# gebegebegebe/onnx-transformer

Measured on AMD Instinct MI355X. Metric: decoded tokens/sec IWSLT14 de-en int8 greedy (batch 32 over 1 GPU, 71 steps), higher is better.
Workload: dtype int8; 1 GPU; cfg2: greedy decode, src<=64 padded to 72, max_len=72, 32 sentences length-sorted over 1 rank(s); global_batch=32, per_gpu_batch=32, seq_len=72, parallelism=sentence-shard x1

## Files before the change

onnx-transformer_amd/csrc/qtx_decode.hip:

```cpp
#include <cstdlib>

#include "qtx_common.h"
#include "qtx_kernels.h"
#include "qtx_knobs.h"

QTX_STAMP_SETTER(decode)

namespace qtx {

__device__ __forceinline__ uint4 unpack_i4(uint2 h) {
  auto sext = [](uint32_t v) { return v | ((v & 0x08080808u) * 0x1Eu); };
  const uint32_t lo0 = sext(h.x & 0x0F0F0F0Fu), hi0 = sext((h.x >> 4) & 0x0F0F0F0Fu);
  const uint32_t lo1 = sext(h.y & 0x0F0F0F0Fu), hi1 = sext((h.y >> 4) & 0x0F0F0F0Fu);
  uint4 o;
  o.x = __builtin_amdgcn_perm(hi0, lo0, 0x05010400u);
  o.y = __builtin_amdgcn_perm(hi0, lo0, 0x07030602u);
  o.z = __builtin_amdgcn_perm(hi1, lo1, 0x05010400u);
  o.w = __builtin_amdgcn_perm(hi1, lo1, 0x07030602u);
  return o;
}

template <int RB, int K, int AMODE, class F>
__device__ __forceinline__ void skinny_prologue(const SkinnyArgs& g, uint8_t* As, float* sas,
                                                int m0, int tid, int wave, int lane,
                                                F&& issue_rest) {
  constexpr int LDA = K + 16;
  constexpr int BM = RB <= 16 ? 16 : 32;
  constexpr int RPW = RB / 4;
  if constexpr (AMODE == A_I8) {
    constexpr int CPR = K / 16, TOT = RB * CPR, NLD = (TOT + 255) / 256;
    uint4 v[NLD];
#pragma unroll
    for (int j = 0; j < NLD; ++j) {
      const int idx = min(tid + 256 * j, TOT - 1), m = min(m0 + idx / CPR, g.M - 1);
      v[j] = ld_at(reinterpret_cast<const uint4*>(g.A), (unsigned)(m * K + 16 * (idx % CPR)));
    }
    issue_rest();
    if (tid < BM) sas[tid] = (tid < RB && m0 + tid < g.M) ? g.sa[m0 + tid] : 0.0f;
#pragma unroll
    for (int j = 0; j < NLD; ++j) {
      const int idx = tid + 256 * j, r = idx / CPR;
      if (TOT % 256 == 0 || idx < TOT)
        *reinterpret_cast<uint4*>(As + r * LDA + 16 * (idx % CPR)) =
            (m0 + r < g.M) ? v[j] : make_uint4(0, 0, 0, 0);
// ... 69 lines not shown
        uint32_t* dst = reinterpret_cast<uint32_t*>(As + r * LDA);
        float tf[4 * NC];
#pragma unroll
        for (int c = 0; c < NC; ++c) {
          tf[4 * c] = t[jb][c].x; tf[4 * c + 1] = t[jb][c].y;
          tf[4 * c + 2] = t[jb][c].z; tf[4 * c + 3] = t[jb][c].w;
        }
        uint32_t qd[NC];
#if defined(QTX_ABL) && (QTX_ABL & 8)
#pragma unroll
        for (int c = 0; c < NC; ++c) qd[c] = __float_as_uint(tf[4 * c] * sc);
#else
        quant_pack<4 * NC>(tf, sc, qd);
#endif
#pragma unroll
        for (int c = 0; c < NC; ++c) dst[lane + 64 * c] = ok ? qd[c] : 0u;
        if (lane == 0) sas[r] = ok ? sc : 0.0f;
      }
    }
  }
}

template <int MF, int RB, int K, int WBITS, int AMODE, int FLAGS>
__global__ __launch_bounds__(256) void k_skinny(SkinnyArgs g) {
  constexpr int BM = 16 * MF;
  static_assert(RB % 4 == 0 && RB <= BM, "rows per block");
  constexpr int KW = K / 4;
  constexpr int NS = KW / 64;
  constexpr int LDA = K + 16;
  __shared__ __attribute__((aligned(16))) uint8_t As[BM * LDA];
  __shared__ float sas[BM];
  __shared__ v4i red[4][MF][64];

  const int tid = threadIdx.x, wave = tid >> 6, lane = tid & 63;
  const int fr = lane & 15, fg = lane >> 4;
  const int n0 = blockIdx.x * 16, m0 = blockIdx.y * RB;

  QTX_STAMP(0);

  const int n = min(n0 + fr, g.N - 1);
  uint4 wf[NS];
  uint2 wp[NS];
  const int col = n0 + fr;
  const bool cok = col < g.N;
  float swc = 0.0f, bc = 0.0f, rv[MF];
  constexpr bool resid = FLAGS & EPI_RESIDUAL;
  auto issue_rest = [&]() {
#pragma unroll
    for (int s = 0; s < NS; ++s) {
      const int k = wave * KW + 64 * s + 16 * fg;
#if defined(QTX_ABL) && (QTX_ABL & 1)
      wf[s] = make_uint4(n + k, k, n, 1); wp[s] = make_uint2(n, k);
#else
      if constexpr (WBITS == 8)
        wf[s] = ld_at(reinterpret_cast<const uint4*>(g.W), (unsigned)(n * (int)g.ldw + k));
      else
        wp[s] = ld_at(reinterpret_cast<const uint2*>(g.W), (unsigned)(n * (int)g.ldw + (k >> 1)));
#endif
    }
    const int cc = min(col, g.N - 1);
    swc = ld_at(g.sw, 4u * cc);
    bc = ld_at(g.bias, 4u * cc);
    if constexpr (resid) {
#pragma unroll
      for (int i = 0; i < MF; ++i) {
        const int row = min(m0 + 16 * i + 4 * fg + wave, g.M - 1);
        rv[i] = ld_at(g.res, 4u * (unsigned)(row * (int)g.ldr + cc));
      }
    }
  };

  skinny_prologue<RB, K, AMODE>(g, As, sas, m0, tid, wave, lane, issue_rest);
  __syncthreads();

  QTX_STAMP(1);
  v4i acc[MF];
#pragma unroll
  for (int i = 0; i < MF; ++i) acc[i] = v4i{0, 0, 0, 0};
#pragma unroll
  for (int s = 0; s < NS; ++s) {
    v4i bfr;
    if constexpr (WBITS == 8) {
      bfr = __builtin_bit_cast(v4i, wf[s]);
    } else {
      bfr = __builtin_bit_cast(v4i, unpack_i4(wp[s]));
    }
    const int k = wave * KW + 64 * s + 16 * fg;
#pragma unroll
    for (int i = 0; i < MF; ++i) {
      const v4i afr = *reinterpret_cast<const v4i*>(As + (16 * i + fr) * LDA + k);
#if defined(QTX_ABL) && (QTX_ABL & 4)
      acc[i] += afr ^ bfr;
// ... 15 lines not shown
      int sum = 0;
#pragma unroll
      for (int w = 0; w < 4; ++w) sum += reinterpret_cast<const int*>(&red[w][i][lane])[e];
      const int r = 16 * i + 4 * fg + e, row = m0 + r;
      const bool ok = cok && r < RB && row < g.M;
      float y = ((float)sum * sas[r]) * swc + bc;
      if constexpr (relu) y = y > 0.0f ? y : 0.0f;
      if constexpr (resid) y = rv[i] + y;
      if (ok) st_at(g.out, 4u * (unsigned)(row * (int)g.ldo + col), y);
      if constexpr (rmax) {
        float am = ok ? fabsf(y) : 0.0f;
        am = fmaxf(am, dpp<0xB1>(am));
        am = fmaxf(am, dpp<0x4E>(am));
        am = fmaxf(am, dpp<0x141>(am));
        am = fmaxf(am, dpp<0x140>(am));
        if (fr == 0 && r < RB && row < g.M) g.pmax_out[(long)blockIdx.x * g.M + row] = am;
      }
    }
  }
  QTX_STAMP(3);
}

template <bool OWN>
__global__ __launch_bounds__(512) void k_skinny8_ffn2(SkinnyArgs g) {
  constexpr int K = 2048, RB = 4, KW = K / 8, NS = KW / 64, LDA = K + 16;
  __shared__ __attribute__((aligned(16))) uint8_t As[16 * LDA];
  __shared__ float sas[16];
  __shared__ v4i red[8][64];
  __shared__ float hmax[8];
  const int tid = threadIdx.x, wave = tid >> 6, lane = tid & 63;
  const int fr = lane & 15, fg = lane >> 4;
  const int n0 = blockIdx.x * 16, m0 = blockIdx.y * RB;
  const int r = wave >> 1, half = wave & 1;
  const int m = min(m0 + r, g.M - 1);
  float4 t[4];
#pragma unroll
  for (int c = 0; c < 4; ++c)
    t[c] = ld_at(reinterpret_cast<const float4*>(g.X), 4u * (unsigned)(m * (int)g.ldx + 4 * (lane + 64 * (4 * half + c))));
  float pm[2] = {0.0f, 0.0f};
  if constexpr (!OWN)
#pragma unroll
    for (int u = 0; u < 2; ++u) pm[u] = ld_at(g.pmax_in, 4u * (unsigned)(min(lane + 64 * u, g.pmax_n - 1) * g.M + m));
  const int n = min(n0 + fr, g.N - 1);
  uint4 wf[NS];
#pragma unroll
  for (int s = 0; s < NS; ++s)
    wf[s] = ld_at(reinterpret_cast<const uint4*>(g.W), (unsigned)(n * (int)g.ldw + wave * KW + 64 * s + 16 * fg));
  const int col = n0 + fr, cc = min(col, g.N - 1);
  const bool cok = col < g.N;
  const float swc = ld_at(g.sw, 4u * cc), bc = ld_at(g.bias, 4u * cc);
  const float rv = ld_at(g.res, 4u * (unsigned)(min(m0 + fg, g.M - 1) * (int)g.ldr + cc));
  {
    const bool ok = m0 + r < g.M;
    float rmax;
    if constexpr (OWN) {
      float lm = 0.0f;
#pragma unroll
      for (int c = 0; c < 4; ++c)
        lm = fmaxf(lm, fmaxf(fmaxf(fabsf(t[c].x), fabsf(t[c].y)), fmaxf(fabsf(t[c].z), fabsf(t[c].w))));
      lm = wave_max(lm);
      if (lane == 0) hmax[wave] = lm;
      __syncthreads();
      rmax = fmaxf(hmax[2 * r], hmax[2 * r + 1]);
    } else {
      rmax = wave_max(fmaxf(pm[0], pm[1]));
    }
    const float sc = quant_scale(rmax, 127.0f);
    float tf[16];
#pragma unroll
    for (int c = 0; c < 4; ++c) {
      tf[4 * c] = t[c].x; tf[4 * c + 1] = t[c].y; tf[4 * c + 2] = t[c].z; tf[4 * c + 3] = t[c].w;
    }
    uint32_t qd[4];
    quant_pack<16>(tf, sc, qd);
// ... 4 lines not shown
  }
  __syncthreads();
  v4i acc = v4i{0, 0, 0, 0};
#pragma unroll
  for (int s = 0; s < NS; ++s) {
    const v4i afr = *reinterpret_cast<const v4i*>(As + fr * LDA + wave * KW + 64 * s + 16 * fg);
    acc = __builtin_amdgcn_mfma_i32_16x16x64_i8(afr, __builtin_bit_cast(v4i, wf[s]), acc, 0, 0, 0);
  }
  red[wave][lane] = acc;
  __syncthreads();
  if (wave != 0) return;
  {
    const int e = fg, src = fr;
    int sum = 0;
#pragma unroll
    for (int w = 0; w < 8; ++w) sum += reinterpret_cast<const int*>(&red[w][src])[e];
    const int row = m0 + e;
    const float y = ((float)sum * sas[e]) * swc + bc;
    if (cok && row < g.M) st_at(g.out, 4u * (unsigned)(row * (int)g.ldo + col), rv + y);
  }
}

template <int RB, int WBITS, int AMODE, int FLAGS>
__global__ __launch_bounds__(256) void k_skinny_wide(SkinnyArgs g) {
  constexpr int K = 512, NS = K / 64, LDA = K + 16;
  static_assert(RB % 4 == 0 && RB <= 16, "rows per block");
  __shared__ __attribute__((aligned(16))) uint8_t As[16 * LDA];
  __shared__ float sas[16];
  constexpr int RPL = RB / 4;
  constexpr bool REMAP = RB == 4 || RB == 8;
  __shared__ v4i tail[REMAP ? 4 : 1][REMAP ? 4 * RB : 1];
  const int tid = threadIdx.x, wave = tid >> 6, lane = tid & 63;
  const int fr = lane & 15, fg = lane >> 4;
  const int n0 = blockIdx.x * 64 + 16 * wave, m0 = blockIdx.y * RB;
  QTX_STAMP(0);
  const int n = min(n0 + fr, g.N - 1);
  uint4 wf[NS];
  uint2 wp[NS];
  const int col = n0 + fr;
  const bool cok = col < g.N;
  constexpr bool resid = FLAGS & EPI_RESIDUAL;
  float swc, bc, rv[4];
  auto issue_rest = [&]() {
#pragma unroll
    for (int s = 0; s < NS; ++s) {
      const int k = 64 * s + 16 * fg;
#if defined(QTX_ABL) && (QTX_ABL & 1)
      wf[s] = make_uint4(n + k, k, n, 1); wp[s] = make_uint2(n, k);
#else
      if constexpr (WBITS == 8)
        wf[s] = ld_at(reinterpret_cast<const uint4*>(g.W), (unsigned)(n * (int)g.ldw + k));
      else
        wp[s] = ld_at(reinterpret_cast<const uint2*>(g.W), (unsigned)(n * (int)g.ldw + (k >> 1)));
#endif
    }
    swc = cok ? ld_at(g.sw, 4u * col) : 0.0f;
    bc = cok ? ld_at(g.bias, 4u * col) : 0.0f;
    if constexpr (RB == 4) {
      rv[0] = (resid && cok && m0 + fg < g.M) ? ld_at(g.res, 4u * (unsigned)((m0 + fg) * (int)g.ldr + col)) : 0.0f;
    } else if constexpr (RB == 8) {
#pragma unroll
      for (int j = 0; j < 2; ++j) {
        const int row = m0 + fg + 4 * j;
        rv[j] = (resid && cok && row < g.M) ? ld_at(g.res, 4u * (unsigned)(row * (int)g.ldr + col)) : 0.0f;
      }
    } else {
#pragma unroll
      for (int e = 0; e < 4; ++e) {
        const int r = 4 * fg + e, row = m0 + r;
        rv[e] = (resid && cok && r < RB && row < g.M) ? ld_at(g.res, 4u * (unsigned)(row * (int)g.ldr + col)) : 0.0f;
      }
    }
  };
  skinny_prologue<RB, K, AMODE>(g, As, sas, m0, tid, wave, lane, issue_rest);
  __syncthreads();
  QTX_STAMP(1);
  v4i acc = v4i{0, 0, 0, 0};
#pragma unroll
  for (int s = 0; s < NS; ++s) {
// ... 58 lines not shown
  for (int e = 0; e < 4; ++e) {
    const int r = 4 * fg + e, row = m0 + r;
    const bool ok = cok && r < RB && row < g.M;
    float y = ((float)acc[e] * sas[r]) * swc + bc;
    if constexpr (relu) y = y > 0.0f ? y : 0.0f;
    if constexpr (resid) y = rv[e] + y;
    if (ok) st_at(g.out, 4u * (unsigned)(row * (int)g.ldo + col), y);
    if constexpr (rmax) {
      float am = ok ? fabsf(y) : 0.0f;
      am = fmaxf(am, dpp<0xB1>(am));
      am = fmaxf(am, dpp<0x4E>(am));
      am = fmaxf(am, dpp<0x141>(am));
      am = fmaxf(am, dpp<0x140>(am));
      if (fr == 0 && r < RB && row < g.M) g.pmax_out[(long)(n0 >> 4) * g.M + row] = am;
    }
  }
  QTX_STAMP(3);
}

template <int RB, int WB, int AM>
hipError_t skinny_wide_flags(const SkinnyArgs& g, hipStream_t st) {
  const dim3 grid(g.N / 64, (g.M + RB - 1) / RB);
  switch (g.flags) {
    case 0: k_skinny_wide<RB, WB, AM, 0><<<grid, 256, 0, st>>>(g); break;
    case EPI_RELU: k_skinny_wide<RB, WB, AM, EPI_RELU><<<grid, 256, 0, st>>>(g); break;
    case EPI_RESIDUAL: k_skinny_wide<RB, WB, AM, EPI_RESIDUAL><<<grid, 256, 0, st>>>(g); break;
    case EPI_RELU | EPI_ROWMAX:
      k_skinny_wide<RB, WB, AM, EPI_RELU | EPI_ROWMAX><<<grid, 256, 0, st>>>(g);
      break;
    default: return hipErrorInvalidValue;
  }
  return hipGetLastError();
}
template <int WB, int AM>
hipError_t skinny_wide_rb(const SkinnyArgs& g, int rb, hipStream_t st) {
  switch (rb) {
    case 4: return skinny_wide_flags<4, WB, AM>(g, st);
    case 8: return skinny_wide_flags<8, WB, AM>(g, st);
    case 16: return skinny_wide_flags<16, WB, AM>(g, st);
    default: return hipErrorInvalidValue;
  }
}

template <int MF, int RB, int K, int WB, int AM>
hipError_t skinny_flags(const SkinnyArgs& g, hipStream_t st) {
  const dim3 grid(g.N / 16, (g.M + RB - 1) / RB);
  switch (g.flags) {
    case 0: k_skinny<MF, RB, K, WB, AM, 0><<<grid, 256, 0, st>>>(g); break;
    case EPI_RELU: k_skinny<MF, RB, K, WB, AM, EPI_RELU><<<grid, 256, 0, st>>>(g); break;
    case EPI_RESIDUAL: k_skinny<MF, RB, K, WB, AM, EPI_RESIDUAL><<<grid, 256, 0, st>>>(g); break;
    case EPI_RELU | EPI_ROWMAX:
      k_skinny<MF, RB, K, WB, AM, EPI_RELU | EPI_ROWMAX><<<grid, 256, 0, st>>>(g);
      break;
    default: return hipErrorInvalidValue;
  }
  return hipGetLastError();
}
template <int K, int WB, int AM>
hipError_t skinny_rb(const SkinnyArgs& g, int rb, hipStream_t st) {
  switch (rb) {
    case 4: return skinny_flags<1, 4, K, WB, AM>(g, st);
    case 8: return skinny_flags<1, 8, K, WB, AM>(g, st);
    case 16: return skinny_flags<1, 16, K, WB, AM>(g, st);
    case 32: return skinny_flags<2, 32, K, WB, AM>(g, st);
    default: return hipErrorInvalidValue;
  }
}
template <int WB>
hipError_t skinny_mode(const SkinnyArgs& g, hipStream_t st) {
  const Knobs& kn = knobs();
  const bool big = g.M >= 96;
  const int wide_env = kn.skinny_wide;
  const bool wide = wide_env < 0 ? ((g.amode == A_LN && g.N >= 1024) || big) : wide_env > 0;
  if (wide && g.K == 512 && g.N % 64 == 0) {
    const int rb = wide_env > 0 && g.M > 4 ? wide_env : (big ? 8 : 4);
    if (g.amode == A_I8) return skinny_wide_rb<WB, A_I8>(g, rb, st);
    if (g.amode == A_LN) return skinny_wide_rb<WB, A_LN>(g, rb, st);
    if (g.amode == A_F32Q) return skinny_wide_rb<WB, A_F32Q>(g, rb, st);
    if (g.amode == A_F32R) return skinny_wide_rb<WB, A_F32R>(g, rb, st);
  }
  if (g.K == 512) {
    const int rb_i8 = kn.rb_i8_512, rb_ln = kn.rb_ln;
    if (g.amode == A_I8) return skinny_rb<512, WB, A_I8>(g, g.M <= 4 ? 4 : rb_i8, st);
    if (g.amode == A_LN) return skinny_rb<512, WB, A_LN>(g, rb_ln, st);
    if (g.amode == A_F32Q) return skinny_rb<512, WB, A_F32Q>(g, g.M <= 4 ? 4 : rb_i8, st);
    if (g.amode == A_F32R) return skinny_rb<512, WB, A_F32R>(g, g.M <= 4 ? 4 : rb_i8, st);
  } else if (g.K == 2048) {
    const int sk8_maxm = kn.skinny8_maxm;
    if (g.M <= sk8_maxm && WB == 8 && g.flags == EPI_RESIDUAL &&
        ((g.amode == A_F32Q && g.pmax_n <= 128) || g.amode == A_F32R)) {
      if (g.amode == A_F32R)
        k_skinny8_ffn2<true><<<dim3(g.N / 16, (g.M + 3) / 4), 512, 0, st>>>(g);
      else
        k_skinny8_ffn2<false><<<dim3(g.N / 16, (g.M + 3) / 4), 512, 0, st>>>(g);
      return hipGetLastError();
    }
    const int rb_i8 = kn.rb_i8_2048 > 0 ? kn.rb_i8_2048 : (big ? 16 : 4);
    const int rb_f = kn.rb_f32q > 0 ? kn.rb_f32q : (g.M >= 192 ? 16 : big ? 8 : 4);
    if (g.amode == A_I8) return skinny_rb<2048, WB, A_I8>(g, rb_i8, st);
    if (g.amode == A_F32Q) return skinny_rb<2048, WB, A_F32Q>(g, rb_f, st);
    if (g.amode == A_F32R) return skinny_rb<2048, WB, A_F32R>(g, rb_f, st);
  }
  return hipErrorInvalidValue;
}

hipError_t launch_skinny(const SkinnyArgs& g, int wbits, hipStream_t st) {
  if (g.M <= 0) return hipSuccess;
  if (g.N % 16) return hipErrorInvalidValue;
  const long lim = 1L << 30;
  if ((long)g.M * (g.ldx > g.K ? g.ldx : g.K) >= lim || (long)g.M * g.ldr >= lim ||
      (long)g.M * g.ldo >= lim || (long)g.N * g.ldw >= lim || (long)g.M * g.pmax_n >= lim)
    return hipErrorInvalidValue;
  if (wbits == 8) return skinny_mode<8>(g, st);
  if (wbits == 4) return skinny_mode<4>(g, st);
  return hipErrorInvalidValue;
}

constexpr int DEC_MAXK = 128;
constexpr int DEC_KST = 20;

template <bool KV_NEW, int NIT>
__global__ __launch_bounds__(64) void k_dec_attn(DecAttnArgs a) {
  __shared__ __attribute__((aligned(16))) uint32_t Ks[DEC_MAXK * DEC_KST];
  __shared__ __attribute__((aligned(16))) uint8_t Vs[DEC_MAXK * 64];
  __shared__ float svs[DEC_MAXK];
  __shared__ __attribute__((aligned(16))) float PS[DEC_MAXK];
  __shared__ __attribute__((aligned(16))) int8_t qs[64];
  const int b = blockIdx.x, h = blockIdx.y, lane = threadIdx.x;
  QTX_STAMP(0);
  const float* yr = a.y + (long)b * a.ldy;
  const int nrows = KV_NEW ? (a.host_step1 > 0 ? a.host_step1 : (int)a.kv_bs) : a.S;
  const long kvb = (long)b * a.kv_bs;
  const long vgb = (long)b * ((a.kv_bs + 3) >> 2);

  float4 yq[2], yk[2], yv[2];
#pragma unroll
  for (int c = 0; c < 2; ++c) {
    yq[c] = *reinterpret_cast<const float4*>(yr + 4 * (lane + 64 * c));
    if constexpr (KV_NEW) {
      yk[c] = *reinterpret_cast<const float4*>(yr + 512 + 4 * (lane + 64 * c));
      yv[c] = *reinterpret_cast<const float4*>(yr + 1024 + 4 * (lane + 64 * c));
    }
  }
  const float q_own = yr[h * 64 + lane];
  const float k_own = KV_NEW ? yr[512 + h * 64 + lane] : 0.0f;
  const float v_own = KV_NEW ? yr[1024 + h * 64 + lane] : 0.0f;
  const int step = !KV_NEW ? 0 : a.host_step1 > 0 ? a.host_step1 - 1 : min(max(*a.step, 0), (int)a.kv_bs - 1);
  const int rsub = lane >> 2, ch = lane & 3;
  const int vg = lane >> 4, vd = 4 * (lane & 15), glast = (nrows - 1) >> 2;
  const int8_t* const kbase = a.kc + kvb * 512 + h * 64;
  const int8_t* const vbase = a.vc + vgb * 2048 + h * 256;
  uint4 kr[NIT], vr[NIT];
#pragma unroll
  for (int i = 0; i < NIT; ++i) {
    const unsigned koff = (unsigned)(min(16 * i + rsub, nrows - 1) * 512 + 16 * ch);
    const unsigned voff = (unsigned)(min(4 * i + vg, glast) * 2048 + 4 * vd);
    kr[i] = __builtin_bit_cast(uint4, __builtin_nontemporal_load(reinterpret_cast<const v4i*>(kbase + koff)));
    vr[i] = __builtin_bit_cast(uint4, __builtin_nontemporal_load(reinterpret_cast<const v4i*>(vbase + voff)));
  }
  const int j0 = min(lane, nrows - 1), j1 = min(lane + 64, nrows - 1);
  const float* const skb = a.skc + kvb;
  const float* const svb = a.svc + kvb;
  float sk0 = skb[(unsigned)j0], sk1 = skb[(unsigned)j1];
  const float sv0 = svb[(unsigned)j0], sv1 = svb[(unsigned)j1];
  bool keep0 = true, keep1 = true;
  if constexpr (!KV_NEW) {
    const uint8_t* const mb = a.mask + (long)b * a.S;
    keep0 = mb[(unsigned)j0] != 0;
    keep1 = mb[(unsigned)j1] != 0;
  }
  int Sk = KV_NEW ? step + 1 : a.S;
  if constexpr (!KV_NEW) {
    const int last = wave_max_i32(max(keep0 && lane < a.S ? lane + 1 : 0,
                                      keep1 && lane + 64 < a.S ? lane + 65 : 0));
    if (last > 0) Sk = last;
  }

  auto amax8 = [](const float4 (&v)[2]) {
    float m = 0.0f;
#pragma unroll
    for (int c = 0; c < 2; ++c)
      m = fmaxf(m, fmaxf(fmaxf(fabsf(v[c].x), fabsf(v[c].y)), fmaxf(fabsf(v[c].z), fabsf(v[c].w))));
    return wave_max(m);
  };
  const float sq = quant_scale(amax8(yq), 127.0f);
  qs[lane] = (int8_t)quant_one(q_own, sq);
  int8_t kq = 0, vq = 0;
  float sk = 0.0f, sv = 0.0f;
  if constexpr (KV_NEW) {
    sk = quant_scale(amax8(yk), 127.0f);
    sv = quant_scale(amax8(yv), 127.0f);
    kq = (int8_t)quant_one(k_own, sk);
    vq = (int8_t)quant_one(v_own, sv);
// ... 95 lines not shown
#pragma unroll
        for (int e = 0; e < 4; ++e) v[4 * q + e] = (float)(int8_t)(vg4[g][q] >> (8 * e));
      const float4 p0 = pg[g][0], p1 = pg[g][1], p2 = pg[g][2], p3 = pg[g][3];
      fmac(c0, p0.x, v[0]);  fmac(c1, p1.x, v[4]);  fmac(c2, p2.x, v[8]);  fmac(c3, p3.x, v[12]);
      fmac(c0, p0.y, v[1]);  fmac(c1, p1.y, v[5]);  fmac(c2, p2.y, v[9]);  fmac(c3, p3.y, v[13]);
      fmac(c0, p0.z, v[2]);  fmac(c1, p1.z, v[6]);  fmac(c2, p2.z, v[10]); fmac(c3, p3.z, v[14]);
      fmac(c0, p0.w, v[3]);  fmac(c1, p1.w, v[7]);  fmac(c2, p2.w, v[11]); fmac(c3, p3.w, v[15]);
    }
  }
  const float acc = (c0 + c1) + (c2 + c3);
  QTX_STAMP(3);

  st_at(a.ctx, 4u * (unsigned)(b * 512 + h * 64 + lane), acc);
  if (a.pmax) {
    const float am = wave_max(fabsf(acc));
    if (lane == 0) a.pmax[(long)h * a.B + b] = am;
  }
  QTX_STAMP(4);
}

template <bool KV_NEW>
hipError_t dec_attn_nit(const DecAttnArgs& a, int B, int nrows, hipStream_t st) {
  const dim3 grid(B, 8), block(64);
  switch ((nrows + 15) / 16) {
    case 1: k_dec_attn<KV_NEW, 1><<<grid, block, 0, st>>>(a); break;
    case 2: k_dec_attn<KV_NEW, 2><<<grid, block, 0, st>>>(a); break;
    case 3: k_dec_attn<KV_NEW, 3><<<grid, block, 0, st>>>(a); break;
    case 4: k_dec_attn<KV_NEW, 4><<<grid, block, 0, st>>>(a); break;
    case 5: k_dec_attn<KV_NEW, 5><<<grid, block, 0, st>>>(a); break;
    case 6: k_dec_attn<KV_NEW, 6><<<grid, block, 0, st>>>(a); break;
    case 7: k_dec_attn<KV_NEW, 7><<<grid, block, 0, st>>>(a); break;
    case 8: k_dec_attn<KV_NEW, 8><<<grid, block, 0, st>>>(a); break;
    default: return hipErrorInvalidValue;
  }
  return hipGetLastError();
}

hipError_t launch_dec_attn(const DecAttnArgs& a, int B, hipStream_t st) {
  if (B <= 0) return hipSuccess;
  if (!a.ctx || a.B != B) return hipErrorInvalidValue;
  if (a.kv_new) {
    if (a.kv_bs <= 0 || a.kv_bs > DEC_MAXK || a.host_step1 < 0 || a.host_step1 > a.kv_bs)
      return hipErrorInvalidValue;
    return dec_attn_nit<true>(a, B, a.host_step1 > 0 ? a.host_step1 : (int)a.kv_bs, st);
  }
  if (a.S <= 0 || a.S > DEC_MAXK) return hipErrorInvalidValue;
  return dec_attn_nit<false>(a, B, a.S, st);
}

__global__ void k_vgroup4(const int8_t* v, long v_ls, int B, int S, int8_t* out, long o_ls) {
  const int G4 = (S + 3) >> 2;
  const long n = (long)B * G4 * 512;
  const long i = (long)blockIdx.x * blockDim.x + threadIdx.x;
  if (i >= n) return;
  const int d = (int)(i & 511);
  const long bg = i >> 9;
  const int g = (int)(bg % G4), b = (int)(bg / G4);
  const int8_t* src = v + (long)blockIdx.y * v_ls;
  uint32_t w = 0;
#pragma unroll
  for (int e = 0; e < 4; ++e) {
    const int j = 4 * g + e;
    const uint32_t byte = j < S ? (uint8_t)src[((long)b * S + j) * 512 + d] : 0u;
// ... 28 lines not shown
  const float sc = quant_scale(fmaxf(fmaxf(wm[0], wm[1]), fmaxf(wm[2], wm[3])), 127.0f);
  float tf[8];
#pragma unroll
  for (int c = 0; c < 2; ++c) {
    tf[4 * c] = t[c].x; tf[4 * c + 1] = t[c].y; tf[4 * c + 2] = t[c].z; tf[4 * c + 3] = t[c].w;
  }
  uint32_t qd[2];
  quant_pack<8>(tf, sc, qd);
  uint32_t* dst = reinterpret_cast<uint32_t*>(q + (long)m * 2048 + 512 * wave);
#pragma unroll
  for (int c = 0; c < 2; ++c) dst[lane + 64 * c] = qd[c];
  if (tid == 0) s[m] = sc;
}

hipError_t launch_quant_h2048(const float* X, long ldx, int M, int8_t* q, float* s,
                              hipStream_t st) {
  if (M <= 0) return hipSuccess;
  k_quant_h2048<<<dim3(M), dim3(256), 0, st>>>(X, ldx, M, q, s);
  return hipGetLastError();
}

constexpr int GEN_Q = 32;

__global__ __launch_bounds__(1024) void k_generator_mfma(const float* x, long ldx, int M,
                                                         const float* ln_a, const float* ln_b,
                                                         const float* Wm, const float* bias,
                                                         int V, float* logits) {
  __shared__ __attribute__((aligned(16))) float X[16][514];
  __shared__ __attribute__((aligned(16))) v4f part[3][4][64];
  const int tid = threadIdx.x, wave = tid >> 6, lane = tid & 63;
  const int fr = lane & 15, fg = lane >> 4;
  const int sw = wave & 3, qq = wave >> 2;
  const unsigned nrb = (unsigned)(M + 15) >> 4, hw = blockIdx.x;
  const int rb = (int)((hw >> 3) % nrb), g = (int)(((hw >> 3) / nrb) * 8 + (hw & 7));
  const int nstrip = (V + 15) / 16, strip = g * 4 + sw;
  if (g * 4 >= nstrip) return;
  const int m0 = rb * 16;
  const int vcol = strip * 16 + fr;
  QTX_STAMP(0);
  constexpr int QQ = GEN_Q / 4;
  const unsigned wo = 16u * (unsigned)((min(strip, nstrip - 1) * GEN_Q + QQ * qq) * 64 + lane);
  float4 wq[QQ];
#pragma unroll
  for (int q = 0; q < QQ; ++q) wq[q] = ld_at(reinterpret_cast<const float4*>(Wm), wo + 1024u * q);
  const float bv = ld_at(bias, 4u * min(vcol, V - 1));
  float xv[1][2][4];
  {
    const int m = min(m0 + wave, M - 1);
#pragma unroll
    for (int c = 0; c < 2; ++c) {
// ... 20 lines not shown
      acc = __builtin_amdgcn_mfma_f32_16x16x4f32(a, b4[e], acc, 0, 0, 0);
    }
  }
  if (qq) part[qq - 1][sw][lane] = acc;
  __syncthreads();
  QTX_STAMP(2);
  if (qq || vcol >= V) return;
  const v4f p1 = part[0][sw][lane], p2 = part[1][sw][lane], p3 = part[2][sw][lane];
#pragma unroll
  for (int e = 0; e < 4; ++e) {
    const int m = m0 + 4 * fg + e;
    if (m < M) st_at(logits, 4u * (unsigned)(m * V + vcol), ((acc[e] + p1[e]) + (p2[e] + p3[e])) + bv);
  }
  QTX_STAMP(3);
}

hipError_t launch_generator_mfma(const float* x, long ldx, int M, const float* ln_a,
                                 const float* ln_b, const float* Wm, const float* b, int V,
                                 float* logits, hipStream_t st) {
  if (M <= 0) return hipSuccess;
  if ((long)M * V >= (1L << 30) || (long)M * ldx >= (1L << 30)) return hipErrorInvalidValue;
  const int ngroup = (V + 63) / 64, nrb = (M + 15) / 16;
  const unsigned grid = 8u * nrb * ((ngroup + 7) / 8);
  k_generator_mfma<<<dim3(grid), dim3(1024), 0, st>>>(x, ldx, M, ln_a, ln_b, Wm, b, V, logits);
  return hipGetLastError();
}

__global__ void k_pack_gen(const float* W, int V, float* out) {
  const long i = (long)blockIdx.x * blockDim.x + threadIdx.x;
  const int nstrip = (V + 15) / 16;
  if (i >= (long)nstrip * GEN_Q * 64) return;
  const int l = (int)(i % 64), q = (int)((i / 64) % GEN_Q), c = (int)(i / (64 * GEN_Q));
  const int v = 16 * c + (l & 15);
  float4 o;
  float* op = reinterpret_cast<float*>(&o);
#pragma unroll
  for (int e = 0; e < 4; ++e) op[e] = v < V ? W[(long)v * 512 + 4 * (4 * q + e) + (l >> 4)] : 0.0f;
  reinterpret_cast<float4*>(out)[i] = o;
}
hipError_t launch_pack_gen(const float* W, int V, float* out, hipStream_t st) {
  const long n = (long)((V + 15) / 16) * GEN_Q * 64;
  k_pack_gen<<<dim3((unsigned)((n + 255) / 256)), dim3(256), 0, st>>>(W, V, out);
  return hipGetLastError();
}

#ifdef QTX_STAMPS
extern "C" int qtx_debug_generator(const float* x, int M, const float* lna, const float* lnb,
// ... 12 lines not shown
  for (int i = ty; i < 32; i += 8)
    if (c0 + i < Cc && r0 + tx < R) out[(long)(c0 + i) * R + r0 + tx] = t[tx][i];
}
hipError_t launch_transpose(const float* in, int R, int Cc, float* out, hipStream_t st) {
  k_transpose<<<dim3((Cc + 31) / 32, (R + 31) / 32), dim3(32, 8), 0, st>>>(in, R, Cc, out);
  return hipGetLastError();
}

constexpr int ARG_T = 1024, ARG_NV = 8, ARG_MAXV = ARG_T * ARG_NV;
constexpr float ARG_DELTA = 4.0e-6f;

__device__ __forceinline__ int wave_sum_i32(int v) {
  auto d = [](int x, auto ctrl) {
    return __builtin_amdgcn_update_dpp(0, x, decltype(ctrl)::value, 0xF, 0xF, true);
  };
  v += d(v, std::integral_constant<int, 0xB1>{});
  v += d(v, std::integral_constant<int, 0x4E>{});
  v += d(v, std::integral_constant<int, 0x141>{});
  v += d(v, std::integral_constant<int, 0x140>{});
  return (__builtin_amdgcn_readlane(v, 0) + __builtin_amdgcn_readlane(v, 16)) +
         (__builtin_amdgcn_readlane(v, 32) + __builtin_amdgcn_readlane(v, 48));
}

__global__ __launch_bounds__(1024) void k_argmax_embed(const float* logits, int V, int64_t* ids,
                                                       long ids_bs, int* step, unsigned* arrive,
                                                       const float* lut, const float* pe,
                                                       int max_pos, float* xnext, int host_s1) {
  __shared__ float Ev[ARG_MAXV];
  __shared__ float redf[16], lse_s;
  __shared__ int redi[16], redc[16], redb[16];
  const int m = blockIdx.x, tid = threadIdx.x, lane = tid & 63, w = tid >> 6;
  QTX_STAMP(0);
  const int s = host_s1 > 0 ? host_s1 - 1 : *step;
  const unsigned xo = 4u * (unsigned)(m * V);
  float4 pe_row = make_float4(0.0f, 0.0f, 0.0f, 0.0f);
  if (tid < 128) pe_row = ld_at(reinterpret_cast<const float4*>(pe), 16u * (unsigned)(min(s + 1, max_pos - 1) * 128 + tid));
  float t[ARG_NV];
#pragma unroll
  for (int i = 0; i < ARG_NV; ++i) t[i] = ld_at(logits, xo + 4u * min(tid + ARG_T * i, V - 1));
  QTX_STAMP(1);
  float lm = -3.0e38f;
  bool nonfin = false, fin = false;
#pragma unroll
  for (int i = 0; i < ARG_NV; ++i)
    if (tid + ARG_T * i < V) {
      lm = fmaxf(lm, t[i]);
      nonfin |= !(t[i] < __builtin_inff());
      fin |= t[i] > -__builtin_inff();
    }
  lm = wave_max(lm);
  const int flags = (__ballot(nonfin) ? 1 : 0) | (__ballot(fin) ? 2 : 0);
  if (lane == 0) { redf[w] = lm; redb[w] = flags; }
  __syncthreads();
  const float mx = wave_max(lane < 16 ? redf[lane] : -3.0e38f);
  int cnt = 0, bi = 0x7fffffff;
#pragma unroll
  for (int i = 0; i < ARG_NV; ++i) {
    const int v = tid + ARG_T * i;
    if (v < V) {
      cnt += t[i] > mx - ARG_DELTA ? 1 : 0;
      if (t[i] == mx && v < bi) bi = v;
    }
// ... 49 lines not shown
  QTX_STAMP(4);
  if (tid < 128) {
    const float sc = 0x1.6a09e6p+4f;
    const float4 e = ld_at(reinterpret_cast<const float4*>(lut), 16u * (unsigned)(id * 128 + tid));
    const float4 q = pe_row;
    st_at(reinterpret_cast<float4*>(xnext), 16u * (unsigned)(m * 128 + tid),
          make_float4(e.x * sc + q.x, e.y * sc + q.y, e.z * sc + q.z, e.w * sc + q.w));
  }
  QTX_STAMP(5);
  if (host_s1 == 0 && tid == 0) {
    const unsigned tk = atomicAdd(arrive, 1u);
    if (tk == gridDim.x - 1) {
      *step = s + 1;
      *arrive = 0u;
    }
  }
}

hipError_t launch_argmax_embed(const float* logits, int M, int V, int64_t* ids, long ids_bs,
                               int* step, unsigned* arrive, const float* lut, const float* pe,
                               int max_pos, float* xnext, hipStream_t st, int host_s1) {
  if (M <= 0) return hipSuccess;
  if (V > ARG_MAXV || host_s1 < 0 || (long)M * V >= (1L << 30)) return hipErrorInvalidValue;
  k_argmax_embed<<<dim3(M), dim3(ARG_T), 0, st>>>(logits, V, ids, ids_bs, step, arrive, lut,
                                                  pe, max_pos, xnext, host_s1);
  return hipGetLastError();
}

}
```

onnx-transformer_amd/qtx/_build.py:

```python
from __future__ import annotations

import os
import shutil
import subprocess

HERE = os.path.dirname(os.path.abspath(__file__))
CSRC = os.path.join(os.path.dirname(HERE), "csrc")
REPO = os.path.dirname(os.path.dirname(HERE))
LIB = os.path.join(HERE, "libqtx.so")
SOURCES = ["qtx_kernels.hip", "qtx_decode.hip", "qtx_gemm.hip", "qtx_wsgemm.hip", "qtx_attn.hip",
           "qtx_ffn.hip", "qtx_api.hip", "qtx_knobs.hip"]
DIAG_SOURCES = ["diag/qtx_wsgemm_diag.hip"]
HEADERS = ["qtx_common.h", "qtx_kernels.h", "qtx_ws.h", "qtx_knobs.h"]

FLAGS = ["--offload-arch=gfx950", "-O3", "-std=c++17", "-fPIC", "-shared",
         "-ffp-contract=off", "-fno-fast-math", "-Wall"]


def hipcc() -> str:
    for cand in (os.environ.get("HIPCC"), shutil.which("hipcc"), "/opt/rocm/bin/hipcc"):
        if cand and os.path.exists(cand):
            return cand
    raise RuntimeError("hipcc not found: the qtx HIP extension cannot be built")


def _inputs():
    files = [os.path.join(CSRC, s) for s in SOURCES + HEADERS]
    files.append(os.path.join(REPO, "include", "qtx.h"))
    files.append(os.path.abspath(__file__))
    return files


def up_to_date() -> bool:
    if not os.path.exists(LIB):
        return False
    t = os.path.getmtime(LIB)
    return all(os.path.getmtime(f) <= t for f in _inputs())


def build(force: bool = False, verbose: bool = False, extra=()) -> str:
    from concurrent.futures import ThreadPoolExecutor
    out = LIB if not extra else LIB.replace(".so", "_diag.so")
    extra = list(extra) + (["-DQTX_DIAG"] if extra and "-DQTX_DIAG" not in extra else [])
    if not force and not extra and up_to_date():
        return LIB
    objdir = os.path.join(HERE, "build_obj")
    os.makedirs(objdir, exist_ok=True)
    cflags = [f for f in FLAGS if f != "-shared"] + list(extra)

    def compile_one(src):
        obj = os.path.join(objdir, os.path.splitext(os.path.basename(src))[0] + ("_x" if extra else "") + ".o")
        cmd = [hipcc(), *cflags, "-c", "-o", obj, os.path.join(CSRC, src)]
        if verbose:
            print(" ".join(cmd), flush=True)
        r = subprocess.run(cmd, capture_output=True, text=True)
        if r.returncode != 0:
            raise RuntimeError(f"hipcc failed on {src} ({r.returncode}):\n{r.stderr[-4000:]}")
        return obj

    srcs = SOURCES + (DIAG_SOURCES if extra else [])
    with ThreadPoolExecutor(max_workers=min(len(srcs), os.cpu_count() or 1)) as ex:
        objs = list(ex.map(compile_one, srcs))
    tmp = out + ".tmp"
    cmd = [hipcc(), "--offload-arch=gfx950", "-shared", "-fPIC", "-o", tmp, *objs]
    r = subprocess.run(cmd, capture_output=True, text=True)
    if r.returncode != 0:
        raise RuntimeError(f"hipcc link failed ({r.returncode}):\n{r.stderr[-4000:]}")
    os.replace(tmp, out)
    return out


if __name__ == "__main__":
    print(build(force=True, verbose=True))
```

Measured before the change: 191,600 tokens/s.

## Preload kernel arguments into SGPRs for decode kernels and reorder early loads

Decode kernels now take their hottest arguments as seven leading 64-bit scalars, and the decode source is built with kernarg preload of 14 dwords. The leading pointers and sizes therefore arrive in SGPRs at wave launch rather than through s_load from the kernarg segment. Argument lists are reordered so the first loads depend only on preloaded values, and sched_barriers push dependent loads such as step, bias and pe later. This targets per-kernel startup latency in a launch-bound decode loop, at the cost of packing/unpacking complexity and reliance on an LLVM option.

```diff
diff --git a/onnx-transformer_amd/csrc/qtx_decode.hip b/onnx-transformer_amd/csrc/qtx_decode.hip
--- a/onnx-transformer_amd/csrc/qtx_decode.hip
+++ b/onnx-transformer_amd/csrc/qtx_decode.hip
@@ -20,6 +20,79 @@
   return o;
 }
 
+struct KaLead { uint64_t w[7]; };
+#define QTX_KA_PARAMS uint64_t ka0, uint64_t ka1, uint64_t ka2, uint64_t ka3, uint64_t ka4, \
+                      uint64_t ka5, uint64_t ka6
+#define QTX_KA_VALS KaLead{{ka0, ka1, ka2, ka3, ka4, ka5, ka6}}
+#define QTX_KA_ARGS(l) (l).w[0], (l).w[1], (l).w[2], (l).w[3], (l).w[4], (l).w[5], (l).w[6]
+template <class L> KaLead ka_pack(const L& l) {
+  static_assert(sizeof(L) == sizeof(KaLead), "a lead block is the 14 preloaded dwords");
+  return __builtin_bit_cast(KaLead, l);
+}
+inline uint64_t ka_int(const void* p) { return (uint64_t)reinterpret_cast<uintptr_t>(p); }
+template <class T> __device__ __forceinline__ T* ka_ptr(uint64_t v) {
+  return (T*)(__attribute__((address_space(1))) T*)v;
+}
+
+template <int AMODE> struct SkLead;
+template <> struct SkLead<A_I8> {
+  uint64_t A; int M, N; uint64_t W; int ldw, ldr; uint64_t sw, bias, res;
+};
+template <> struct SkLead<A_LN> {
+  uint64_t X; int M, ldx; uint64_t ln_a, ln_b, W; int ldw, N; uint64_t sw;
+};
+template <> struct SkLead<A_F32Q> {
+  uint64_t X; int M, ldx; uint64_t pmax_in; int pmax_n, ldw; uint64_t W; int N, ldo; uint64_t sw;
+};
+template <> struct SkLead<A_F32R> {
+  uint64_t X; int M, ldx; uint64_t W; int ldw, N; uint64_t sw, res; int ldr, ldo;
+};
+struct SkTail {
+  const float* sa; const float* bias; const float* res; float* out; float* pmax_out;
+  int ldo, ldr;
+};
+
+template <int AMODE> KaLead sk_lead(const SkinnyArgs& g) {
+  SkLead<AMODE> l{};
+  l.M = g.M; l.N = g.N; l.W = ka_int(g.W); l.ldw = (int)g.ldw; l.sw = ka_int(g.sw);
+  if constexpr (AMODE == A_I8) {
+    l.A = ka_int(g.A); l.ldr = (int)g.ldr; l.bias = ka_int(g.bias); l.res = ka_int(g.res);
+  } else {
+    l.X = ka_int(g.X); l.ldx = (int)g.ldx;
+    if constexpr (AMODE == A_LN) { l.ln_a = ka_int(g.ln_a); l.ln_b = ka_int(g.ln_b); }
+    if constexpr (AMODE == A_F32Q) { l.pmax_in = ka_int(g.pmax_in); l.pmax_n = g.pmax_n; l.ldo = (int)g.ldo; }
+    if constexpr (AMODE == A_F32R) { l.res = ka_int(g.res); l.ldr = (int)g.ldr; l.ldo = (int)g.ldo; }
+  }
+  return ka_pack(l);
+}
+inline SkTail sk_tail(const SkinnyArgs& g) {
+  return SkTail{g.sa, g.bias, g.res, g.out, g.pmax_out, (int)g.ldo, (int)g.ldr};
+}
+template <int AMODE>
+__device__ __forceinline__ SkinnyArgs sk_args(const KaLead& k, const SkTail& t) {
+  const SkLead<AMODE> l = __builtin_bit_cast(SkLead<AMODE>, k);
+  SkinnyArgs g{};
+  g.sa = t.sa; g.bias = t.bias; g.res = t.res; g.out = t.out; g.pmax_out = t.pmax_out;
+  g.ldo = t.ldo; g.ldr = t.ldr;
+  g.M = l.M; g.N = l.N; g.W = ka_ptr<const int8_t>(l.W); g.ldw = l.ldw;
+  g.sw = ka_ptr<const float>(l.sw);
+  if constexpr (AMODE == A_I8) {
+    g.A = ka_ptr<const int8_t>(l.A); g.ldr = l.ldr; g.bias = ka_ptr<const float>(l.bias);
+    g.res = ka_ptr<const float>(l.res);
+  } else {
+    g.X = ka_ptr<const float>(l.X); g.ldx = l.ldx;
+    if constexpr (AMODE == A_LN) { g.ln_a = ka_ptr<const float>(l.ln_a); g.ln_b = ka_ptr<const float>(l.ln_b); }
+    if constexpr (AMODE == A_F32Q) { g.pmax_in = ka_ptr<const float>(l.pmax_in); g.pmax_n = l.pmax_n; g.ldo = l.ldo; }
+    if constexpr (AMODE == A_F32R) { g.res = ka_ptr<const float>(l.res); g.ldr = l.ldr; g.ldo = l.ldo; }
+  }
+  return g;
+}
+#define QTX_SK_LAUNCH(AM, grid, block, ...)                                          \
+  do {                                                                               \
+    const KaLead ka_l_ = sk_lead<AM>(g);                                             \
+    __VA_ARGS__<<<grid, block, 0, st>>>(QTX_KA_ARGS(ka_l_), sk_tail(g));             \
+  } while (0)
+
 template <int RB, int K, int AMODE, class F>
 __device__ __forceinline__ void skinny_prologue(const SkinnyArgs& g, uint8_t* As, float* sas,
                                                 int m0, int tid, int wave, int lane,
@@ -135,7 +208,8 @@
 }
 
 template <int MF, int RB, int K, int WBITS, int AMODE, int FLAGS>
-__global__ __launch_bounds__(256) void k_skinny(SkinnyArgs g) {
+__global__ __launch_bounds__(256) void k_skinny(QTX_KA_PARAMS, SkTail kt) {
+  const SkinnyArgs g = sk_args<AMODE>(QTX_KA_VALS, kt);
   constexpr int BM = 16 * MF;
   static_assert(RB % 4 == 0 && RB <= BM, "rows per block");
   constexpr int KW = K / 4;
@@ -173,7 +247,7 @@
     }
     const int cc = min(col, g.N - 1);
     swc = ld_at(g.sw, 4u * cc);
-    bc = ld_at(g.bias, 4u * cc);
+    __builtin_amdgcn_sched_barrier(0);
     if constexpr (resid) {
 #pragma unroll
       for (int i = 0; i < MF; ++i) {
@@ -181,6 +255,7 @@
         rv[i] = ld_at(g.res, 4u * (unsigned)(row * (int)g.ldr + cc));
       }
     }
+    bc = ld_at(g.bias, 4u * cc);
   };
 
   skinny_prologue<RB, K, AMODE>(g, As, sas, m0, tid, wave, lane, issue_rest);
@@ -242,7 +317,8 @@
 }
 
 template <bool OWN>
-__global__ __launch_bounds__(512) void k_skinny8_ffn2(SkinnyArgs g) {
+__global__ __launch_bounds__(512) void k_skinny8_ffn2(QTX_KA_PARAMS, SkTail kt) {
+  const SkinnyArgs g = sk_args<OWN ? A_F32R : A_F32Q>(QTX_KA_VALS, kt);
   constexpr int K = 2048, RB = 4, KW = K / 8, NS = KW / 64, LDA = K + 16;
   __shared__ __attribute__((aligned(16))) uint8_t As[16 * LDA];
   __shared__ float sas[16];
@@ -268,8 +344,10 @@
     wf[s] = ld_at(reinterpret_cast<const uint4*>(g.W), (unsigned)(n * (int)g.ldw + wave * KW + 64 * s + 16 * fg));
   const int col = n0 + fr, cc = min(col, g.N - 1);
   const bool cok = col < g.N;
-  const float swc = ld_at(g.sw, 4u * cc), bc = ld_at(g.bias, 4u * cc);
+  const float swc = ld_at(g.sw, 4u * cc);
+  __builtin_amdgcn_sched_barrier(0);
   const float rv = ld_at(g.res, 4u * (unsigned)(min(m0 + fg, g.M - 1) * (int)g.ldr + cc));
+  const float bc = ld_at(g.bias, 4u * cc);
   {
     const bool ok = m0 + r < g.M;
     float rmax;
@@ -320,7 +398,8 @@
 }
 
 template <int RB, int WBITS, int AMODE, int FLAGS>
-__global__ __launch_bounds__(256) void k_skinny_wide(SkinnyArgs g) {
+__global__ __launch_bounds__(256) void k_skinny_wide(QTX_KA_PARAMS, SkTail kt) {
+  const SkinnyArgs g = sk_args<AMODE>(QTX_KA_VALS, kt);
   constexpr int K = 512, NS = K / 64, LDA = K + 16;
   static_assert(RB % 4 == 0 && RB <= 16, "rows per block");
   __shared__ __attribute__((aligned(16))) uint8_t As[16 * LDA];
@@ -353,6 +432,7 @@
 #endif
     }
     swc = cok ? ld_at(g.sw, 4u * col) : 0.0f;
+    __builtin_amdgcn_sched_barrier(0);
     bc = cok ? ld_at(g.bias, 4u * col) : 0.0f;
     if constexpr (RB == 4) {
       rv[0] = (resid && cok && m0 + fg < g.M) ? ld_at(g.res, 4u * (unsigned)((m0 + fg) * (int)g.ldr + col)) : 0.0f;
@@ -457,11 +537,11 @@
 hipError_t skinny_wide_flags(const SkinnyArgs& g, hipStream_t st) {
   const dim3 grid(g.N / 64, (g.M + RB - 1) / RB);
   switch (g.flags) {
-    case 0: k_skinny_wide<RB, WB, AM, 0><<<grid, 256, 0, st>>>(g); break;
-    case EPI_RELU: k_skinny_wide<RB, WB, AM, EPI_RELU><<<grid, 256, 0, st>>>(g); break;
-    case EPI_RESIDUAL: k_skinny_wide<RB, WB, AM, EPI_RESIDUAL><<<grid, 256, 0, st>>>(g); break;
+    case 0: QTX_SK_LAUNCH(AM, grid, 256, k_skinny_wide<RB, WB, AM, 0>); break;
+    case EPI_RELU: QTX_SK_LAUNCH(AM, grid, 256, k_skinny_wide<RB, WB, AM, EPI_RELU>); break;
+    case EPI_RESIDUAL: QTX_SK_LAUNCH(AM, grid, 256, k_skinny_wide<RB, WB, AM, EPI_RESIDUAL>); break;
     case EPI_RELU | EPI_ROWMAX:
-      k_skinny_wide<RB, WB, AM, EPI_RELU | EPI_ROWMAX><<<grid, 256, 0, st>>>(g);
+      QTX_SK_LAUNCH(AM, grid, 256, k_skinny_wide<RB, WB, AM, EPI_RELU | EPI_ROWMAX>);
       break;
     default: return hipErrorInvalidValue;
   }
@@ -481,11 +561,11 @@
 hipError_t skinny_flags(const SkinnyArgs& g, hipStream_t st) {
   const dim3 grid(g.N / 16, (g.M + RB - 1) / RB);
   switch (g.flags) {
-    case 0: k_skinny<MF, RB, K, WB, AM, 0><<<grid, 256, 0, st>>>(g); break;
-    case EPI_RELU: k_skinny<MF, RB, K, WB, AM, EPI_RELU><<<grid, 256, 0, st>>>(g); break;
-    case EPI_RESIDUAL: k_skinny<MF, RB, K, WB, AM, EPI_RESIDUAL><<<grid, 256, 0, st>>>(g); break;
+    case 0: QTX_SK_LAUNCH(AM, grid, 256, k_skinny<MF, RB, K, WB, AM, 0>); break;
+    case EPI_RELU: QTX_SK_LAUNCH(AM, grid, 256, k_skinny<MF, RB, K, WB, AM, EPI_RELU>); break;
+    case EPI_RESIDUAL: QTX_SK_LAUNCH(AM, grid, 256, k_skinny<MF, RB, K, WB, AM, EPI_RESIDUAL>); break;
     case EPI_RELU | EPI_ROWMAX:
-      k_skinny<MF, RB, K, WB, AM, EPI_RELU | EPI_ROWMAX><<<grid, 256, 0, st>>>(g);
+      QTX_SK_LAUNCH(AM, grid, 256, k_skinny<MF, RB, K, WB, AM, EPI_RELU | EPI_ROWMAX>);
       break;
     default: return hipErrorInvalidValue;
   }
@@ -525,9 +605,9 @@
     if (g.M <= sk8_maxm && WB == 8 && g.flags == EPI_RESIDUAL &&
         ((g.amode == A_F32Q && g.pmax_n <= 128) || g.amode == A_F32R)) {
       if (g.amode == A_F32R)
-        k_skinny8_ffn2<true><<<dim3(g.N / 16, (g.M + 3) / 4), 512, 0, st>>>(g);
+        QTX_SK_LAUNCH(A_F32R, dim3(g.N / 16, (g.M + 3) / 4), 512, k_skinny8_ffn2<true>);
       else
-        k_skinny8_ffn2<false><<<dim3(g.N / 16, (g.M + 3) / 4), 512, 0, st>>>(g);
+        QTX_SK_LAUNCH(A_F32Q, dim3(g.N / 16, (g.M + 3) / 4), 512, k_skinny8_ffn2<false>);
       return hipGetLastError();
     }
     const int rb_i8 = kn.rb_i8_2048 > 0 ? kn.rb_i8_2048 : (big ? 16 : 4);
@@ -554,8 +634,37 @@
 constexpr int DEC_MAXK = 128;
 constexpr int DEC_KST = 20;
 
+template <bool KV_NEW> struct DaLead;
+template <> struct DaLead<true> {
+  uint64_t y; int ldy, kv_bs; uint64_t kc, vc, skc, svc; int host_step1, zero;
+};
+template <> struct DaLead<false> {
+  uint64_t y; int ldy, kv_bs; uint64_t kc, vc, skc, svc; int S, zero;
+};
+struct DaTail { const int* step; const uint8_t* mask; float* ctx; float* pmax; int B; };
+
+template <bool KV_NEW> KaLead da_lead(const DecAttnArgs& a) {
+  DaLead<KV_NEW> l{};
+  l.y = ka_int(a.y); l.ldy = (int)a.ldy; l.kv_bs = (int)a.kv_bs;
+  l.kc = ka_int(a.kc); l.vc = ka_int(a.vc); l.skc = ka_int(a.skc); l.svc = ka_int(a.svc);
+  if constexpr (KV_NEW) l.host_step1 = a.host_step1; else l.S = a.S;
+  return ka_pack(l);
+}
+template <bool KV_NEW>
+__device__ __forceinline__ DecAttnArgs da_args(const KaLead& k, const DaTail& t) {
+  const DaLead<KV_NEW> l = __builtin_bit_cast(DaLead<KV_NEW>, k);
+  DecAttnArgs a{};
+  a.y = ka_ptr<const float>(l.y); a.ldy = l.ldy; a.kv_bs = l.kv_bs;
+  a.kc = ka_ptr<int8_t>(l.kc); a.vc = ka_ptr<int8_t>(l.vc);
+  a.skc = ka_ptr<float>(l.skc); a.svc = ka_ptr<float>(l.svc);
+  if constexpr (KV_NEW) a.host_step1 = l.host_step1; else a.S = l.S;
+  a.step = t.step; a.mask = t.mask; a.ctx = t.ctx; a.pmax = t.pmax; a.B = t.B;
+  return a;
+}
+
 template <bool KV_NEW, int NIT>
-__global__ __launch_bounds__(64) void k_dec_attn(DecAttnArgs a) {
+__global__ __launch_bounds__(64) void k_dec_attn(QTX_KA_PARAMS, DaTail kt) {
+  const DecAttnArgs a = da_args<KV_NEW>(QTX_KA_VALS, kt);
   __shared__ __attribute__((aligned(16))) uint32_t Ks[DEC_MAXK * DEC_KST];
   __shared__ __attribute__((aligned(16))) uint8_t Vs[DEC_MAXK * 64];
   __shared__ float svs[DEC_MAXK];
@@ -564,9 +673,6 @@
   const int b = blockIdx.x, h = blockIdx.y, lane = threadIdx.x;
   QTX_STAMP(0);
   const float* yr = a.y + (long)b * a.ldy;
-  const int nrows = KV_NEW ? (a.host_step1 > 0 ? a.host_step1 : (int)a.kv_bs) : a.S;
-  const long kvb = (long)b * a.kv_bs;
-  const long vgb = (long)b * ((a.kv_bs + 3) >> 2);
 
   float4 yq[2], yk[2], yv[2];
 #pragma unroll
@@ -580,7 +686,10 @@
   const float q_own = yr[h * 64 + lane];
   const float k_own = KV_NEW ? yr[512 + h * 64 + lane] : 0.0f;
   const float v_own = KV_NEW ? yr[1024 + h * 64 + lane] : 0.0f;
-  const int step = !KV_NEW ? 0 : a.host_step1 > 0 ? a.host_step1 - 1 : min(max(*a.step, 0), (int)a.kv_bs - 1);
+  __builtin_amdgcn_sched_barrier(0);
+  const int nrows = KV_NEW ? (a.host_step1 > 0 ? a.host_step1 : (int)a.kv_bs) : a.S;
+  const long kvb = (long)b * a.kv_bs;
+  const long vgb = (long)b * ((a.kv_bs + 3) >> 2);
   const int rsub = lane >> 2, ch = lane & 3;
   const int vg = lane >> 4, vd = 4 * (lane & 15), glast = (nrows - 1) >> 2;
   const int8_t* const kbase = a.kc + kvb * 512 + h * 64;
@@ -604,6 +713,7 @@
     keep0 = mb[(unsigned)j0] != 0;
     keep1 = mb[(unsigned)j1] != 0;
   }
+  const int step = !KV_NEW ? 0 : a.host_step1 > 0 ? a.host_step1 - 1 : min(max(*a.step, 0), (int)a.kv_bs - 1);
   int Sk = KV_NEW ? step + 1 : a.S;
   if constexpr (!KV_NEW) {
     const int last = wave_max_i32(max(keep0 && lane < a.S ? lane + 1 : 0,
@@ -745,15 +855,17 @@
 template <bool KV_NEW>
 hipError_t dec_attn_nit(const DecAttnArgs& a, int B, int nrows, hipStream_t st) {
   const dim3 grid(B, 8), block(64);
+  const KaLead l = da_lead<KV_NEW>(a);
+  const DaTail t{a.step, a.mask, a.ctx, a.pmax, a.B};
   switch ((nrows + 15) / 16) {
-    case 1: k_dec_attn<KV_NEW, 1><<<grid, block, 0, st>>>(a); break;
-    case 2: k_dec_attn<KV_NEW, 2><<<grid, block, 0, st>>>(a); break;
-    case 3: k_dec_attn<KV_NEW, 3><<<grid, block, 0, st>>>(a); break;
-    case 4: k_dec_attn<KV_NEW, 4><<<grid, block, 0, st>>>(a); break;
-    case 5: k_dec_attn<KV_NEW, 5><<<grid, block, 0, st>>>(a); break;
-    case 6: k_dec_attn<KV_NEW, 6><<<grid, block, 0, st>>>(a); break;
-    case 7: k_dec_attn<KV_NEW, 7><<<grid, block, 0, st>>>(a); break;
-    case 8: k_dec_attn<KV_NEW, 8><<<grid, block, 0, st>>>(a); break;
+    case 1: k_dec_attn<KV_NEW, 1><<<grid, block, 0, st>>>(QTX_KA_ARGS(l), t); break;
+    case 2: k_dec_attn<KV_NEW, 2><<<grid, block, 0, st>>>(QTX_KA_ARGS(l), t); break;
+    case 3: k_dec_attn<KV_NEW, 3><<<grid, block, 0, st>>>(QTX_KA_ARGS(l), t); break;
+    case 4: k_dec_attn<KV_NEW, 4><<<grid, block, 0, st>>>(QTX_KA_ARGS(l), t); break;
+    case 5: k_dec_attn<KV_NEW, 5><<<grid, block, 0, st>>>(QTX_KA_ARGS(l), t); break;
+    case 6: k_dec_attn<KV_NEW, 6><<<grid, block, 0, st>>>(QTX_KA_ARGS(l), t); break;
+    case 7: k_dec_attn<KV_NEW, 7><<<grid, block, 0, st>>>(QTX_KA_ARGS(l), t); break;
+    case 8: k_dec_attn<KV_NEW, 8><<<grid, block, 0, st>>>(QTX_KA_ARGS(l), t); break;
     default: return hipErrorInvalidValue;
   }
   return hipGetLastError();
@@ -762,6 +874,7 @@
 hipError_t launch_dec_attn(const DecAttnArgs& a, int B, hipStream_t st) {
   if (B <= 0) return hipSuccess;
   if (!a.ctx || a.B != B) return hipErrorInvalidValue;
+  if (a.ldy < 0 || a.ldy >= (1L << 31) || a.kv_bs >= (1L << 31)) return hipErrorInvalidValue;
   if (a.kv_new) {
     if (a.kv_bs <= 0 || a.kv_bs > DEC_MAXK || a.host_step1 < 0 || a.host_step1 > a.kv_bs)
       return hipErrorInvalidValue;
@@ -836,10 +949,10 @@
 
 constexpr int GEN_Q = 32;
 
-__global__ __launch_bounds__(1024) void k_generator_mfma(const float* x, long ldx, int M,
-                                                         const float* ln_a, const float* ln_b,
-                                                         const float* Wm, const float* bias,
-                                                         int V, float* logits) {
+__global__ __launch_bounds__(1024) void k_generator_mfma(const float* Wm, int V, int M,
+                                                         const float* bias, const float* x,
+                                                         long ldx, const float* ln_a,
+                                                         const float* ln_b, float* logits) {
   __shared__ __attribute__((aligned(16))) float X[16][514];
   __shared__ __attribute__((aligned(16))) v4f part[3][4][64];
   const int tid = threadIdx.x, wave = tid >> 6, lane = tid & 63;
@@ -906,7 +1019,7 @@
   if ((long)M * V >= (1L << 30) || (long)M * ldx >= (1L << 30)) return hipErrorInvalidValue;
   const int ngroup = (V + 63) / 64, nrb = (M + 15) / 16;
   const unsigned grid = 8u * nrb * ((ngroup + 7) / 8);
-  k_generator_mfma<<<dim3(grid), dim3(1024), 0, st>>>(x, ldx, M, ln_a, ln_b, Wm, b, V, logits);
+  k_generator_mfma<<<dim3(grid), dim3(1024), 0, st>>>(Wm, V, M, b, x, ldx, ln_a, ln_b, logits);
   return hipGetLastError();
 }
 
@@ -965,22 +1078,24 @@
          (__builtin_amdgcn_readlane(v, 32) + __builtin_amdgcn_readlane(v, 48));
 }
 
-__global__ __launch_bounds__(1024) void k_argmax_embed(const float* logits, int V, int64_t* ids,
-                                                       long ids_bs, int* step, unsigned* arrive,
-                                                       const float* lut, const float* pe,
-                                                       int max_pos, float* xnext, int host_s1) {
+__global__ __launch_bounds__(1024) void k_argmax_embed(const float* logits, int V, int host_s1,
+                                                       int* step, const float* pe,
+                                                       const float* lut, int max_pos,
+                                                       long ids_bs, int64_t* ids,
+                                                       unsigned* arrive, float* xnext) {
   __shared__ float Ev[ARG_MAXV];
   __shared__ float redf[16], lse_s;
   __shared__ int redi[16], redc[16], redb[16];
   const int m = blockIdx.x, tid = threadIdx.x, lane = tid & 63, w = tid >> 6;
   QTX_STAMP(0);
+  const unsigned xo = 4u * (unsigned)(m * V);
+  float t[ARG_NV];
+#pragma unroll
+  for (int i = 0; i < ARG_NV; ++i) t[i] = ld_at(logits, xo + 4u * min(tid + ARG_T * i, V - 1));
+  __builtin_amdgcn_sched_barrier(0);
   const int s = host_s1 > 0 ? host_s1 - 1 : *step;
-  const unsigned xo = 4u * (unsigned)(m * V);
   float4 pe_row = make_float4(0.0f, 0.0f, 0.0f, 0.0f);
   if (tid < 128) pe_row = ld_at(reinterpret_cast<const float4*>(pe), 16u * (unsigned)(min(s + 1, max_pos - 1) * 128 + tid));
-  float t[ARG_NV];
-#pragma unroll
-  for (int i = 0; i < ARG_NV; ++i) t[i] = ld_at(logits, xo + 4u * min(tid + ARG_T * i, V - 1));
   QTX_STAMP(1);
   float lm = -3.0e38f;
   bool nonfin = false, fin = false;
@@ -1076,8 +1191,8 @@
                                int max_pos, float* xnext, hipStream_t st, int host_s1) {
   if (M <= 0) return hipSuccess;
   if (V > ARG_MAXV || host_s1 < 0 || (long)M * V >= (1L << 30)) return hipErrorInvalidValue;
-  k_argmax_embed<<<dim3(M), dim3(ARG_T), 0, st>>>(logits, V, ids, ids_bs, step, arrive, lut,
-                                                  pe, max_pos, xnext, host_s1);
+  k_argmax_embed<<<dim3(M), dim3(ARG_T), 0, st>>>(logits, V, host_s1, step, pe, lut, max_pos,
+                                                  ids_bs, ids, arrive, xnext);
   return hipGetLastError();
 }
 
diff --git a/onnx-transformer_amd/qtx/_build.py b/onnx-transformer_amd/qtx/_build.py
--- a/onnx-transformer_amd/qtx/_build.py
+++ b/onnx-transformer_amd/qtx/_build.py
@@ -15,6 +15,11 @@
 
 FLAGS = ["--offload-arch=gfx950", "-O3", "-std=c++17", "-fPIC", "-shared",
          "-ffp-contract=off", "-fno-fast-math", "-Wall"]
+SOURCE_FLAGS = {"qtx_decode.hip": ["-mllvm", "-amdgpu-kernarg-preload-count=14"]}
+
+
+def compile_flags(src: str, extra=()) -> list:
+    return [f for f in FLAGS if f != "-shared"] + SOURCE_FLAGS.get(os.path.basename(src), []) + list(extra)
 
 
 def hipcc() -> str:
@@ -46,11 +51,10 @@
         return LIB
     objdir = os.path.join(HERE, "build_obj")
     os.makedirs(objdir, exist_ok=True)
-    cflags = [f for f in FLAGS if f != "-shared"] + list(extra)
 
     def compile_one(src):
         obj = os.path.join(objdir, os.path.splitext(os.path.basename(src))[0] + ("_x" if extra else "") + ".o")
-        cmd = [hipcc(), *cflags, "-c", "-o", obj, os.path.join(CSRC, src)]
+        cmd = [hipcc(), *compile_flags(src, extra), "-c", "-o", obj, os.path.join(CSRC, src)]
         if verbose:
             print(" ".join(cmd), flush=True)
         r = subprocess.run(cmd, capture_output=True, text=True)
```

Result: faster. 195,400 tokens/s (median of 6 runs) (+2.0%).
